# a16z/jolt

Measured on AMD Instinct MI355X. Metric: prover trace cycles/sec (sha3-shaped synthetic trace, sumcheck + HyperKZG hot path), higher is better.
Workload: dtype u256 (BN254 Fr / Fq, 8x u32 Montgomery limbs; integer, bit-exact)

## Files before the change

### jolt_amd/csrc/rw_matrix.hip

```cpp
#include <algorithm>
#include <vector>

#include "ctx.hpp"
#include "ints.hpp"
#include "onehot.hpp"
#include "poly_kernels.hip.h"

using namespace jolt;

int32_t jolt_internal_table_new(jolt_ctx* ctx, size_t len, jolt_table** out);
int32_t jolt_internal_bind(jolt_ctx* ctx, jolt_table* const* tables, size_t k, const Fr& r, int32_t order);
int32_t jolt_internal_eq_levels(jolt_ctx* ctx, const Fr* r, size_t n, const Fr& scale, std::vector<jolt_table*>* levels);
int32_t jolt_internal_ensure_scratch(jolt_ctx* ctx, size_t partials, size_t results);

namespace {

constexpr uint64_t kNoAccess = 0xFFFFFFFFFFFFFFFFull;

struct RwArrays {
    uint64_t* key;
    uint64_t *prev_u, *next_u;
    Fr *prev_f, *next_f;
    Fr *val, *ra;
    Fr* wa;
// ... 144 lines not shown
        sm[threadIdx.x] = v;
        __syncthreads();
        for (int off = 1; off < kBlock; off <<= 1) {
            uint64_t t = (int)threadIdx.x >= off ? sm[threadIdx.x - off] : 0ull;
            __syncthreads();
            sm[threadIdx.x] += t;
            __syncthreads();
        }
        if (i < nblocks) sums[i] = carry + sm[threadIdx.x] - v;
        __syncthreads();
        if (threadIdx.x == kBlock - 1) carry += sm[threadIdx.x];
        __syncthreads();
    }
    if (threadIdx.x == 0) total[0] = carry;
}
__global__ __launch_bounds__(kBlock) void k_scan_add(uint64_t* __restrict__ out, uint32_t n, const uint64_t* __restrict__ block_sums) {
    const uint32_t base = (blockIdx.x * kBlock + threadIdx.x) * kScanItems;
    const uint64_t add_ = block_sums[blockIdx.x];
#pragma unroll
    for (int k = 0; k < kScanItems; ++k)
        if (base + k < n) out[base + k] += add_;
}

__global__ __launch_bounds__(kBlock) void k_rw_cycle_match(const uint64_t* __restrict__ key, uint32_t n, uint32_t* __restrict__ sib_lb, uint32_t* __restrict__ matched,
                                                           uint64_t* __restrict__ flags) {
    uint32_t i = blockIdx.x * kBlock + threadIdx.x;
    if (i >= n) return;
    const uint64_t k = key[i], want = k ^ (1ull << 32);
    const uint32_t lb = lower_bound_near(key, n, want, i);
    const bool m = lb < n && key[lb] == want;
    const bool even = ((k >> 32) & 1) == 0;
    sib_lb[i] = lb;
    matched[i] = m ? 1u : 0u;
    flags[i] = ((even || !m) ? 1ull : 0ull) | ((even && m) ? (1ull << 32) : 0ull);
}

template <bool REG>
__global__ __launch_bounds__(kBlock) void k_rw_cycle_round(RwArrays a, uint32_t n, const uint32_t* __restrict__ sib_lb, const uint32_t* __restrict__ matched,
                                                           const Fr* __restrict__ inc, const Fr* __restrict__ e_out, const Fr* __restrict__ e_in, int in_bits, Fr gamma,
                                                           Fr* __restrict__ partials) {
    Fr acc[2] = {Fr::zero(), Fr::zero()};
    const uint32_t stride = gridDim.x * kBlock;
    for (uint32_t i = blockIdx.x * kBlock + threadIdx.x; i < n; i += stride) {
        const uint64_t k = a.key[i];
        const uint32_t row = (uint32_t)(k >> 32);
        const bool even = (row & 1) == 0, m = matched[i] != 0;
        if (!even && m) continue;
        const uint32_t pair = row >> 1;
        const Fr inc0 = ld_fr(inc + 2 * (size_t)pair), inc1 = sub(ld_fr(inc + 2 * (size_t)pair + 1), inc0);
        const Fr ra = ld_fr(a.ra + i), val = ld_fr(a.val + i);
        Fr q0, q1;
        if constexpr (REG) {
            const Fr wa = ld_fr(a.wa + i);
            if (even) {
                Fr ra_slope, wa_slope, val_slope;
                if (m) {
                    const uint32_t o = sib_lb[i];
// ... 17 lines not shown
            if (m) {
                const uint32_t o = sib_lb[i];
                ra_slope = sub(ld_fr(a.ra + o), ra);
                val_slope = sub(ld_fr(a.val + o), val);
            } else {
                ra_slope = neg(ra);
                val_slope = sub(fr_from_u64(a.next_u[i]), val);
            }
            q0 = mul(ra, slope_term(val, inc0, gamma));
            q1 = mul(ra_slope, slope_term(val_slope, inc1, gamma));
        } else {
            q0 = Fr::zero();
            q1 = mul(ra, slope_term(sub(val, fr_from_u64(a.prev_u[i])), inc1, gamma));
        }
        const Fr head = mul(ld_fr(e_out + (pair >> in_bits)), ld_fr(e_in + (pair & ((1u << in_bits) - 1))));
        acc[0] = add(acc[0], mul(head, q0));
        acc[1] = add(acc[1], mul(head, q1));
    }
    block_reduce_store<2>(acc, partials);
}

template <bool REG>
__global__ __launch_bounds__(kBlock) void k_rw_cycle_bind(RwArrays a, uint32_t n, const uint32_t* __restrict__ sib_lb, const uint32_t* __restrict__ matched,
                                                          const uint64_t* __restrict__ scan, Fr r, int shifted, RwArrays o) {
    uint32_t i = blockIdx.x * kBlock + threadIdx.x;
    if (i >= n) return;
    const uint64_t k = a.key[i];
    const uint32_t row = (uint32_t)(k >> 32), col = (uint32_t)k;
    const bool even = (row & 1) == 0, m = matched[i] != 0;
    if (!even && m) return;
    const uint64_t gkey = (uint64_t)(row & ~1u) << 32;
    const uint32_t gs = lower_bound_near(a.key, n, gkey, i), os = lower_bound_near(a.key, n, gkey | (1ull << 32), i);
    const uint64_t s_gs = gs < n ? scan[gs] : 0;
    const uint32_t out_base = (uint32_t)s_gs, m_gs = (uint32_t)(s_gs >> 32);
    const uint32_t lb = sib_lb[i];
    uint32_t pos;
    if (even) pos = out_base + (i - gs) + (lb - os) - ((uint32_t)(scan[i] >> 32) - m_gs);
    else pos = out_base + (i - os) + (lb - gs) - ((lb < n ? (uint32_t)(scan[lb] >> 32) : 0u) - m_gs);
    const Fr ra = ld_fr(a.ra + i), val = ld_fr(a.val + i);
    Fr nra, nval;
    uint64_t np, nn;
    auto lerp = [&](const Fr& lo, const Fr& hi) { return bind_pair(lo, hi, r, shifted); };
    if (even && m) {
        nra = lerp(ra, ld_fr(a.ra + lb));
        nval = lerp(val, ld_fr(a.val + lb));
        np = a.prev_u[i];
        nn = a.next_u[lb];
    } else if (even) {
        nra = lerp(ra, Fr::zero());
        nval = lerp(val, fr_from_u64(a.next_u[i]));
        np = a.prev_u[i];
        nn = a.next_u[i];
    } else {
        nra = lerp(Fr::zero(), ra);
        nval = lerp(fr_from_u64(a.prev_u[i]), val);
        np = a.prev_u[i];
        nn = a.next_u[i];
    }
    o.key[pos] = ((uint64_t)(row >> 1) << 32) | col;
    o.prev_u[pos] = np;
    o.next_u[pos] = nn;
    st_fr(o.ra + pos, nra);
    st_fr(o.val + pos, nval);
    if constexpr (REG) {
        const Fr wa = ld_fr(a.wa + i);
        st_fr(o.wa + pos, (even && m) ? lerp(wa, ld_fr(a.wa + lb)) : (even ? lerp(wa, Fr::zero()) : lerp(Fr::zero(), wa)));
    }
}

__global__ __launch_bounds__(kBlock) void k_rw_to_address_major(RwArrays a, uint32_t n) {
    uint32_t i = blockIdx.x * kBlock + threadIdx.x;
    if (i >= n) return;
    a.key[i] = (uint32_t)a.key[i];
    st_fr(a.prev_f + i, fr_from_u64(a.prev_u[i]));
    st_fr(a.next_f + i, fr_from_u64(a.next_u[i]));
}

__device__ __forceinline__ bool adr_partner(const uint64_t* __restrict__ key, uint32_t n, uint32_t i, uint32_t& other) {
    const uint64_t c = key[i];
    if ((c & 1) == 0) { other = i + 1; return i + 1 < n && key[i + 1] == c + 1; }
    other = i - 1;
    return i > 0 && key[i - 1] == c - 1;
}
__global__ __launch_bounds__(kBlock) void k_rw_address_flags(const uint64_t* __restrict__ key, uint32_t n, uint64_t* __restrict__ flags) {
    uint32_t i = blockIdx.x * kBlock + threadIdx.x;
    if (i >= n) return;
    uint32_t o;
    const bool m = adr_partner(key, n, i, o);
    flags[i] = ((key[i] & 1) == 0 || !m) ? 1ull : 0ull;
}
__global__ __launch_bounds__(kBlock) void k_rw_address_round(RwArrays a, uint32_t n, const Fr* __restrict__ val_init, const Fr* __restrict__ inc_scalar, Fr eq_eval,
                                                             Fr gamma, Fr* __restrict__ partials) {
    Fr acc[2] = {Fr::zero(), Fr::zero()};
    const Fr inc = ld_fr(inc_scalar);
    const uint32_t stride = gridDim.x * kBlock;
    for (uint32_t i = blockIdx.x * kBlock + threadIdx.x; i < n; i += stride) {
        uint32_t o;
        const bool m = adr_partner(a.key, n, i, o);
        const uint64_t c = a.key[i];
        const bool even = (c & 1) == 0;
        if (!even && m) continue;
        const Fr ra = ld_fr(a.ra + i), val = ld_fr(a.val + i);
        Fr s0, s2;
        if (even) {
            Fr ra2, val2;
            if (m) {
                const Fr ora = ld_fr(a.ra + o), oval = ld_fr(a.val + o);
                ra2 = sub(add(ora, ora), ra);
                val2 = sub(add(oval, oval), val);
            } else {
                const Fr cp = ld_fr(val_init + (c | 1));
                ra2 = neg(ra);
                val2 = sub(add(cp, cp), val);
            }
            s0 = mul(mul(eq_eval, ra), slope_term(val, inc, gamma));
            s2 = mul(mul(eq_eval, ra2), slope_term(val2, inc, gamma));
        } else {
            const Fr cp = ld_fr(val_init + (c & ~1ull));
            s0 = Fr::zero();
            s2 = mul(mul(eq_eval, add(ra, ra)), slope_term(sub(add(val, val), cp), inc, gamma));
        }
        acc[0] = add(acc[0], s0);
        acc[1] = add(acc[1], s2);
    }
    block_reduce_store<2>(acc, partials);
}
__global__ __launch_bounds__(kBlock) void k_rw_address_bind(RwArrays a, uint32_t n, const Fr* __restrict__ val_init, const uint64_t* __restrict__ scan, Fr r, int shifted,
                                                            RwArrays o) {
    uint32_t i = blockIdx.x * kBlock + threadIdx.x;
    if (i >= n) return;
    uint32_t p;
    const bool m = adr_partner(a.key, n, i, p);
    const uint64_t c = a.key[i];
    const bool even = (c & 1) == 0;
    if (!even && m) return;
    const uint32_t pos = (uint32_t)scan[i];
    auto lerp = [&](const Fr& lo, const Fr& hi) { return bind_pair(lo, hi, r, shifted); };
    const Fr ra = ld_fr(a.ra + i), val = ld_fr(a.val + i), pv = ld_fr(a.prev_f + i), nx = ld_fr(a.next_f + i);
    Fr nra, nval, npv, nnx;
    if (even && m) {
        nra = lerp(ra, ld_fr(a.ra + p));
        nval = lerp(val, ld_fr(a.val + p));
        npv = lerp(pv, ld_fr(a.prev_f + p));
        nnx = lerp(nx, ld_fr(a.next_f + p));
    } else if (even) {
        const Fr cp = ld_fr(val_init + (c | 1));
        nra = lerp(ra, Fr::zero());
        nval = lerp(val, cp);
        npv = lerp(pv, cp);
        nnx = lerp(nx, cp);
    } else {
        const Fr cp = ld_fr(val_init + (c & ~1ull));
        nra = lerp(Fr::zero(), ra);
        nval = lerp(cp, val);
        npv = lerp(cp, pv);
        nnx = lerp(cp, nx);
    }
    o.key[pos] = c >> 1;
    st_fr(o.ra + pos, nra);
    st_fr(o.val + pos, nval);
    st_fr(o.prev_f + pos, npv);
    st_fr(o.next_f + pos, nnx);
}

}

struct jolt_rw_matrix {
    jolt_ctx* ctx = nullptr;
    size_t log_t = 0, log_k = 0, round = 0;
    uint32_t n = 0, cap = 0;
    void* block = nullptr;
    RwArrays st[2];
    int cur = 0;
    uint32_t *sib_lb = nullptr, *matched = nullptr;
    uint64_t *flags = nullptr, *scan = nullptr, *block_sums = nullptr, *total = nullptr;
    uint64_t* h_total = nullptr;
    bool match_valid = false;
    bool registers = false;
    bool hold_row = false;
    std::vector<Fr> reg_ra, reg_wa, reg_val;
    Fr inc_scalar;
    jolt_table *inc = nullptr, *val_init = nullptr;
    Fr gamma;
    std::vector<Fr> w;
    Fr current_scalar;
    size_t out_len = 0, in_len = 0, e_out_bits = 0, e_in_bits = 0;
    std::vector<jolt_table*> e_out_cache, e_in_cache;
};

static int32_t rw_scan(jolt_rw_matrix* m, uint32_t n) {
    jolt_ctx* ctx = m->ctx;
    const uint32_t per = kBlock * kScanItems, nblocks = std::max<uint32_t>(1, (n + per - 1) / per);
    hipLaunchKernelGGL(k_scan_blocks, dim3(nblocks), dim3(kBlock), 0, ctx->stream, (const uint64_t*)m->flags, n, m->scan, m->block_sums);
    hipLaunchKernelGGL(k_scan_sums, dim3(1), dim3(kBlock), 0, ctx->stream, m->block_sums, nblocks, m->total);
    hipLaunchKernelGGL(k_scan_add, dim3(nblocks), dim3(kBlock), 0, ctx->stream, m->scan, n, (const uint64_t*)m->block_sums);
    JOLT_HIP_TRY(ctx, hipGetLastError());
    return JOLT_OK;
}
static int32_t rw_read_total(jolt_rw_matrix* m, uint32_t* out) {
    jolt_ctx* ctx = m->ctx;
    JOLT_HIP_TRY(ctx, hipMemcpyAsync(m->h_total, m->total, 8, hipMemcpyDeviceToHost, ctx->stream));
    JOLT_HIP_TRY(ctx, hipStreamSynchronize(ctx->stream));
    *out = (uint32_t)*m->h_total;
    return JOLT_OK;
}
static unsigned rw_grid(uint32_t n) { return std::max<unsigned>(1, (n + kBlock - 1) / kBlock); }
constexpr uint32_t kRwRoundMult = 4;

extern "C" int32_t jolt_rw_matrix_destroy(jolt_rw_matrix* m) {
    if (!m) return JOLT_OK;
    jolt_ctx* ctx = m->ctx;
    if (m->block) jolt_internal_dev_free(ctx, m->block);
    if (m->h_total) (void)hipHostFree(m->h_total);
    if (m->inc) jolt_table_free(ctx, m->inc);
    if (m->val_init) jolt_table_free(ctx, m->val_init);
    for (jolt_table* t : m->e_out_cache) jolt_table_free(ctx, t);
    for (jolt_table* t : m->e_in_cache) jolt_table_free(ctx, t);
    delete m;
    return JOLT_OK;
}

static int32_t rw_create_impl(jolt_ctx* ctx, const uint64_t* addresses, const uint64_t* pre_values, const uint64_t* post_values, bool resident, uint32_t resident_cap,
                              size_t cycles, const jolt_table* inc, const jolt_table* val_init, const jolt_fr_t* tau_low, const jolt_fr_t* gamma, jolt_rw_matrix** out) {
    if (!ctx || !addresses || !pre_values || !post_values || !inc || !val_init || !tau_low || !gamma || !out) return JOLT_ERR_INVALID_ARG;
    if (cycles < 2 || (cycles & (cycles - 1)) || cycles > ((size_t)1 << 31) || inc->len != cycles) return JOLT_ERR_SIZE_MISMATCH;
    const size_t K = val_init->len;
    if (K == 0 || (K & (K - 1)) || K > ((size_t)1 << 32)) return JOLT_ERR_SIZE_MISMATCH;
    for (size_t j = 0; j < cycles && !resident; ++j)
        if (addresses[j] != kNoAccess && addresses[j] >= K) { ctx->last_error = "RAM address outside the address space"; return JOLT_ERR_INVALID_ARG; }
    jolt_rw_matrix* m = new (std::nothrow) jolt_rw_matrix();
// ... 36 lines not shown
    if (s == JOLT_OK && hipHostMalloc((void**)&m->h_total, 64, hipHostMallocDefault) != hipSuccess) s = JOLT_ERR_HIP;
    if (s != JOLT_OK) { jolt_rw_matrix_destroy(m); return s; }
    char* base = (char*)m->block;
    for (int b = 0; b < 2; ++b) {
        m->st[b].key = (uint64_t*)(base + o_st[b][0]); m->st[b].prev_u = (uint64_t*)(base + o_st[b][1]); m->st[b].next_u = (uint64_t*)(base + o_st[b][2]);
        m->st[b].prev_f = (Fr*)(base + o_st[b][3]); m->st[b].next_f = (Fr*)(base + o_st[b][4]); m->st[b].val = (Fr*)(base + o_st[b][5]); m->st[b].ra = (Fr*)(base + o_st[b][6]);
        m->st[b].wa = (Fr*)(base + o_st[b][7]);
    }
    m->sib_lb = (uint32_t*)(base + o_sib); m->matched = (uint32_t*)(base + o_match); m->flags = (uint64_t*)(base + o_flags); m->scan = (uint64_t*)(base + o_scan);
    m->block_sums = (uint64_t*)(base + o_bs); m->total = (uint64_t*)(base + o_total);
    const uint64_t *d_addr = addresses, *d_pre = pre_values, *d_post = post_values;
    hipError_t e = hipSuccess;
    if (!resident) {
        uint64_t* up = (uint64_t*)(base + o_up);
        d_addr = up; d_pre = up + cycles; d_post = up + 2 * cycles;
        e = hipMemcpyAsync(up, addresses, cycles * 8, hipMemcpyHostToDevice, ctx->stream);
        if (e == hipSuccess) e = hipMemcpyAsync(up + cycles, pre_values, cycles * 8, hipMemcpyHostToDevice, ctx->stream);
        if (e == hipSuccess) e = hipMemcpyAsync(up + 2 * cycles, post_values, cycles * 8, hipMemcpyHostToDevice, ctx->stream);
    }
    if (e == hipSuccess) {
        hipLaunchKernelGGL(k_rw_access_flags, dim3(rw_grid(T)), dim3(kBlock), 0, ctx->stream, (const uint64_t*)d_addr, T, m->flags);
        e = hipGetLastError();
    }
    if (e == hipSuccess) s = rw_scan(m, T);
    if (e == hipSuccess && s == JOLT_OK) {
        hipLaunchKernelGGL(k_rw_build, dim3(rw_grid(T)), dim3(kBlock), 0, ctx->stream, (const uint64_t*)d_addr, (const uint64_t*)d_pre, (const uint64_t*)d_post, T,
                           (const uint64_t*)m->scan, m->st[0]);
        e = hipGetLastError();
    }
    if (e == hipSuccess && !resident) e = hipStreamSynchronize(ctx->stream);
    if (e != hipSuccess || s != JOLT_OK) {
        if (e != hipSuccess) { ctx->last_error = std::string("rw matrix: ") + hipGetErrorString(e); s = JOLT_ERR_HIP; }
        jolt_rw_matrix_destroy(m);
        return s;
    }
    m->n = cap;
    *out = m;
    return JOLT_OK;
}
extern "C" int32_t jolt_rw_matrix_create(jolt_ctx* ctx, const uint64_t* addresses, const uint64_t* pre_values, const uint64_t* post_values, size_t cycles,
                                         const jolt_table* inc, const jolt_table* val_init, const jolt_fr_t* tau_low, const jolt_fr_t* gamma, jolt_rw_matrix** out) {
    return rw_create_impl(ctx, addresses, pre_values, post_values, false, 0, cycles, inc, val_init, tau_low, gamma, out);
}
__global__ __launch_bounds__(kBlock) void k_rw_count_accesses(const uint64_t* __restrict__ addresses, uint32_t cycles, uint64_t K, uint32_t* __restrict__ counters) {
    __shared__ uint32_t s_hit[kBlock / 64], s_bad[kBlock / 64];
    uint32_t hit = 0, bad = 0;
    for (uint32_t j = blockIdx.x * kBlock + threadIdx.x; j < cycles; j += gridDim.x * kBlock) {
// ... 23 lines not shown
    if (cycles < 2 || cycles > ((size_t)1 << 31)) return JOLT_ERR_SIZE_MISMATCH;
    uint32_t* d_counters = nullptr;
    JOLT_TRY(jolt_internal_dev_alloc(ctx, 256, (void**)&d_counters));
    uint32_t h_counters[2] = {0, 0};
    hipError_t e = hipMemsetAsync(d_counters, 0, 8, ctx->stream);
    if (e == hipSuccess) {
        hipLaunchKernelGGL(k_rw_count_accesses, dim3(std::min<uint32_t>(rw_grid((uint32_t)cycles), (uint32_t)ctx->num_cus * 8)), dim3(kBlock), 0, ctx->stream, (const uint64_t*)addresses->data, (uint32_t)cycles,
                           (uint64_t)val_init->len, d_counters);
        e = hipGetLastError();
    }
    if (e == hipSuccess) e = hipMemcpyAsync(h_counters, d_counters, 8, hipMemcpyDeviceToHost, ctx->stream);
    if (e == hipSuccess) e = hipStreamSynchronize(ctx->stream);
    jolt_internal_dev_free(ctx, d_counters);
    if (e != hipSuccess) { ctx->last_error = std::string("rw matrix: ") + hipGetErrorString(e); return JOLT_ERR_HIP; }
    if (h_counters[1]) { ctx->last_error = "RAM address outside the address space"; return JOLT_ERR_INVALID_ARG; }
    return rw_create_impl(ctx, (const uint64_t*)addresses->data, (const uint64_t*)pre_values->data, (const uint64_t*)post_values->data, true, h_counters[0], cycles, inc,
                          val_init, tau_low, gamma, out);
}

static int32_t rw_ingest(jolt_rw_matrix* m, const Fr& r) {
    jolt_ctx* ctx = m->ctx;
    const int shifted = fr_low_limbs_zero(r) ? 1 : 0;
    RwArrays &a = m->st[m->cur], &o = m->st[1 - m->cur];
    if (m->round < m->log_t) {
        if (m->n) {
            if (!m->match_valid) {
                hipLaunchKernelGGL(k_rw_cycle_match, dim3(rw_grid(m->n)), dim3(kBlock), 0, ctx->stream, (const uint64_t*)a.key, m->n, m->sib_lb, m->matched, m->flags);
                JOLT_HIP_TRY(ctx, hipGetLastError());
            }
            JOLT_TRY(rw_scan(m, m->n));
            if (m->registers)
                hipLaunchKernelGGL(k_rw_cycle_bind<true>, dim3(rw_grid(m->n)), dim3(kBlock), 0, ctx->stream, a, m->n, (const uint32_t*)m->sib_lb, (const uint32_t*)m->matched,
                                   (const uint64_t*)m->scan, r, shifted, o);
            else
                hipLaunchKernelGGL(k_rw_cycle_bind<false>, dim3(rw_grid(m->n)), dim3(kBlock), 0, ctx->stream, a, m->n, (const uint32_t*)m->sib_lb, (const uint32_t*)m->matched,
                                   (const uint64_t*)m->scan, r, shifted, o);
            JOLT_HIP_TRY(ctx, hipGetLastError());
            JOLT_TRY(rw_read_total(m, &m->n));
            m->cur = 1 - m->cur;
        }
        m->match_valid = false;
        JOLT_TRY(jolt_internal_bind(ctx, &m->inc, 1, r, JOLT_ORDER_LOW_TO_HIGH));
        {
            const size_t nvar = m->log_t;
            size_t current_index = nvar - m->round;
            const Fr p = m->w[current_index - 1], prod = mul(p, r);
            m->current_scalar = mul(m->current_scalar, add(add(sub(sub(Fr::one(), p), r), prod), prod));
            current_index -= 1;
            if (nvar / 2 < current_index && m->e_in_bits > 0) m->e_in_bits -= 1;
            else if (0 < current_index && m->e_out_bits > 0) m->e_out_bits -= 1;
        }
        if (m->round == m->log_t - 1 && m->hold_row) {
        } else if (m->round == m->log_t - 1 && m->registers) {
            const size_t K = (size_t)1 << m->log_k;
            m->reg_ra.assign(K, Fr::zero());
            m->reg_wa.assign(K, Fr::zero());
            m->reg_val.assign(K, Fr::zero());
            const uint32_t n = m->n;
            if (n > K) { ctx->last_error = "registers matrix: more cells than registers after the cycle rounds"; return JOLT_ERR_INVALID_ARG; }
            std::vector<uint64_t> key(n);
            std::vector<Fr> ra(n), wa(n), val(n);
            const RwArrays& c = m->st[m->cur];
            hipError_t first = hipSuccess;
            auto copy = [&](void* dst, const void* src, size_t bytes) {
// ... 7 lines not shown
                copy(val.data(), c.val, (size_t)n * sizeof(Fr));
            }
            copy(&m->inc_scalar, m->inc->data(), sizeof(Fr));
            const hipError_t sync = hipStreamSynchronize(ctx->stream);
            JOLT_HIP_TRY(ctx, first);
            JOLT_HIP_TRY(ctx, sync);
            for (uint32_t i = 0; i < n; ++i) {
                const uint32_t col = (uint32_t)key[i];
                if ((key[i] >> 32) != 0 || col >= K) { ctx->last_error = "registers matrix: a cell outside the single bound row"; return JOLT_ERR_INVALID_ARG; }
                m->reg_ra[col] = ra[i]; m->reg_wa[col] = wa[i]; m->reg_val[col] = val[i];
            }
        } else if (m->round == m->log_t - 1 && m->n) {
            hipLaunchKernelGGL(k_rw_to_address_major, dim3(rw_grid(m->n)), dim3(kBlock), 0, ctx->stream, m->st[m->cur], m->n);
            JOLT_HIP_TRY(ctx, hipGetLastError());
        }
    } else if (m->registers) {
        for (std::vector<Fr>* t : {&m->reg_ra, &m->reg_wa, &m->reg_val}) {
            const size_t half = t->size() / 2;
            for (size_t y = 0; y < half; ++y) (*t)[y] = add((*t)[2 * y], mul(r, sub((*t)[2 * y + 1], (*t)[2 * y])));
            t->resize(half);
        }
    } else {
        if (m->n) {
            hipLaunchKernelGGL(k_rw_address_flags, dim3(rw_grid(m->n)), dim3(kBlock), 0, ctx->stream, (const uint64_t*)a.key, m->n, m->flags);
            JOLT_HIP_TRY(ctx, hipGetLastError());
            JOLT_TRY(rw_scan(m, m->n));
            hipLaunchKernelGGL(k_rw_address_bind, dim3(rw_grid(m->n)), dim3(kBlock), 0, ctx->stream, a, m->n, (const Fr*)m->val_init->data(), (const uint64_t*)m->scan, r,
                               shifted, o);
            JOLT_HIP_TRY(ctx, hipGetLastError());
            JOLT_TRY(rw_read_total(m, &m->n));
            m->cur = 1 - m->cur;
        }
        JOLT_TRY(jolt_internal_bind(ctx, &m->val_init, 1, r, JOLT_ORDER_LOW_TO_HIGH));
    }
    m->round += 1;
    return JOLT_OK;
}

extern "C" int32_t jolt_rw_matrix_prove_round(jolt_rw_matrix* m, const jolt_fr_t* bind, jolt_fr_t* evals_out, jolt_fr_t* aux_out) {
    if (!m || !evals_out) return JOLT_ERR_INVALID_ARG;
    jolt_ctx* ctx = m->ctx;
    if (m->registers) { ctx->last_error = "a registers handle: use jolt_registers_rw_prove_round (this entry point ignores the wa column)"; return JOLT_ERR_INVALID_ARG; }
    if (bind) {
        Fr r = fr_from_abi(bind);
        JOLT_REQUIRE(ctx, fr_is_canonical(r), "bind challenge is not a canonical Fr");
        if (m->round >= m->log_t + m->log_k) { ctx->last_error = "rw matrix already fully bound"; return JOLT_ERR_INVALID_ARG; }
        JOLT_TRY(rw_ingest(m, r));
    }
    if (m->round >= m->log_t + m->log_k) { ctx->last_error = "prove_round on a fully bound rw matrix"; return JOLT_ERR_INVALID_ARG; }
    const int grid = (int)std::max<uint32_t>(1, std::min<uint32_t>((m->n + kBlock - 1) / kBlock, (uint32_t)ctx->num_cus * kRwRoundMult));
    JOLT_TRY(jolt_internal_ensure_scratch(ctx, (size_t)grid * 2 + 8, 8));
    RwArrays& a = m->st[m->cur];
    Fr zero = Fr::zero();
    if (m->round < m->log_t) {
        if (m->n && !m->match_valid) {
            hipLaunchKernelGGL(k_rw_cycle_match, dim3(rw_grid(m->n)), dim3(kBlock), 0, ctx->stream, (const uint64_t*)a.key, m->n, m->sib_lb, m->matched, m->flags);
            JOLT_HIP_TRY(ctx, hipGetLastError());
            m->match_valid = true;
        }
        hipLaunchKernelGGL(k_rw_cycle_round<false>, dim3(grid), dim3(kBlock), 0, ctx->stream, a, m->n, (const uint32_t*)m->sib_lb, (const uint32_t*)m->matched,
                           (const Fr*)m->inc->data(), (const Fr*)m->e_out_cache[m->e_out_bits]->data(), (const Fr*)m->e_in_cache[m->e_in_bits]->data(), (int)m->e_in_bits,
                           m->gamma, ctx->d_partials);
        if (aux_out) {
            fr_to_abi(&aux_out[0], m->current_scalar);
            fr_to_abi(&aux_out[1], m->w[m->log_t - m->round - 1]);
            fr_to_abi(&aux_out[2], zero);
        }
    } else {
        hipLaunchKernelGGL(k_rw_address_round, dim3(grid), dim3(kBlock), 0, ctx->stream, a, m->n, (const Fr*)m->val_init->data(), (const Fr*)m->inc->data(),
                           m->current_scalar, m->gamma, ctx->d_partials);
        if (aux_out) for (int k = 0; k < 3; ++k) fr_to_abi(&aux_out[k], zero);
    }
    JOLT_HIP_TRY(ctx, hipGetLastError());
    hipLaunchKernelGGL(k_reduce_partials, dim3(1), dim3(kBlock), 0, ctx->stream, (const Fr*)ctx->d_partials, grid, 2, ctx->d_results);
    JOLT_HIP_TRY(ctx, hipGetLastError());
    JOLT_HIP_TRY(ctx, hipMemcpyAsync(ctx->h_results, ctx->d_results, 2 * sizeof(Fr), hipMemcpyDeviceToHost, ctx->stream));
    JOLT_HIP_TRY(ctx, hipStreamSynchronize(ctx->stream));
    std::memcpy(evals_out, ctx->h_results, 2 * sizeof(Fr));
    return JOLT_OK;
}

extern "C" int32_t jolt_rw_matrix_finish(jolt_rw_matrix* m, const jolt_fr_t* bind) {
    if (!m || !bind) return JOLT_ERR_INVALID_ARG;
    Fr r = fr_from_abi(bind);
    JOLT_REQUIRE(m->ctx, fr_is_canonical(r), "bind challenge is not a canonical Fr");
    if (m->round + 1 != m->log_t + m->log_k) { m->ctx->last_error = "finish_rounds before the last round"; return JOLT_ERR_INVALID_ARG; }
    return rw_ingest(m, r);
}

extern "C" int32_t jolt_rw_matrix_final_values(jolt_rw_matrix* m, jolt_fr_t* out) {
    if (!m || !out) return JOLT_ERR_INVALID_ARG;
    jolt_ctx* ctx = m->ctx;
    if (m->registers) { ctx->last_error = "a registers handle: use jolt_registers_rw_final_values (no val_init column here)"; return JOLT_ERR_INVALID_ARG; }
    if (m->round != m->log_t + m->log_k) return JOLT_ERR_NOT_FULLY_BOUND;
    Fr vals[3];
    if (m->n) {
        JOLT_HIP_TRY(ctx, hipMemcpyAsync(&vals[0], m->st[m->cur].ra, sizeof(Fr), hipMemcpyDeviceToHost, ctx->stream));
        JOLT_HIP_TRY(ctx, hipMemcpyAsync(&vals[1], m->st[m->cur].val, sizeof(Fr), hipMemcpyDeviceToHost, ctx->stream));
    } else {
        vals[0] = Fr::zero();
        JOLT_HIP_TRY(ctx, hipMemcpyAsync(&vals[1], m->val_init->data(), sizeof(Fr), hipMemcpyDeviceToHost, ctx->stream));
// ... 189 lines not shown
    while (((size_t)1 << m->log_k) < K) m->log_k++;
    m->gamma = fr_from_abi(gamma);
    m->w.resize(m->log_t);
    for (size_t i = 0; i < m->log_t; ++i) m->w[i] = fr_from_abi(&r_cycle[i]);
    m->current_scalar = Fr::one();
    int32_t s = fr_is_canonical(m->gamma) ? JOLT_OK : JOLT_ERR_INVALID_ARG;
    for (size_t i = 0; i < m->log_t && s == JOLT_OK; ++i) if (!fr_is_canonical(m->w[i])) s = JOLT_ERR_INVALID_ARG;
    const size_t split = m->log_t / 2, head_len = m->log_t - 1;
    m->out_len = std::min(split, head_len);
    m->in_len = head_len - m->out_len;
    m->e_out_bits = m->out_len;
    m->e_in_bits = m->in_len;
    if (s == JOLT_OK) s = jolt_internal_eq_levels(ctx, m->w.data(), m->out_len, Fr::one(), &m->e_out_cache);
    if (s == JOLT_OK) s = jolt_internal_eq_levels(ctx, m->w.data() + m->out_len, m->in_len, Fr::one(), &m->e_in_cache);
    if (s == JOLT_OK) s = jolt_table_clone(ctx, inc, &m->inc);
    const uint32_t T = (uint32_t)cycles;
    const size_t scan_len0 = T;
    uint64_t *d_flags0 = nullptr;
    if (s == JOLT_OK) s = jolt_internal_dev_alloc(ctx, (2 * scan_len0 + ((scan_len0 + kBlock * kScanItems - 1) / (kBlock * kScanItems) + 1) + 32) * 8, (void**)&d_flags0);
    if (s == JOLT_OK && hipHostMalloc((void**)&m->h_total, 64, hipHostMallocDefault) != hipSuccess) s = JOLT_ERR_HIP;
    if (s != JOLT_OK) { if (d_flags0) jolt_internal_dev_free(ctx, d_flags0); jolt_rw_matrix_destroy(m); return s; }
    m->flags = d_flags0; m->scan = d_flags0 + scan_len0; m->block_sums = m->scan + scan_len0; m->total = m->block_sums + ((scan_len0 + kBlock * kScanItems - 1) / (kBlock * kScanItems) + 1);
    hipLaunchKernelGGL(k_reg_count, dim3(rw_grid(T)), dim3(kBlock), 0, ctx->stream, (const uint8_t*)regs->idx, regs->wide, T, m->flags);
    s = hipGetLastError() == hipSuccess ? rw_scan(m, T) : JOLT_ERR_HIP;
    uint32_t cap = 0;
    if (s == JOLT_OK) s = rw_read_total(m, &cap);
    if (s != JOLT_OK) { jolt_internal_dev_free(ctx, d_flags0); m->flags = m->scan = m->block_sums = m->total = nullptr; jolt_rw_matrix_destroy(m); return s; }
    m->cap = std::max<uint32_t>(cap, 1);
    const size_t scan_len = std::max<size_t>(T, m->cap);
    size_t off = 0;
    auto take = [&](size_t bytes) { size_t o = off; off += (bytes + 255) & ~(size_t)255; return o; };
    size_t o_st[2][6];
    for (int b = 0; b < 2; ++b) {
        o_st[b][0] = take((size_t)m->cap * 8); o_st[b][1] = take((size_t)m->cap * 8); o_st[b][2] = take((size_t)m->cap * 8);
        o_st[b][3] = take((size_t)m->cap * 32); o_st[b][4] = take((size_t)m->cap * 32); o_st[b][5] = take((size_t)m->cap * 32);
    }
    const size_t o_sib = take((size_t)m->cap * 4), o_match = take((size_t)m->cap * 4), o_flags = take(scan_len * 8), o_scan = take(scan_len * 8),
                 o_bs = take(((scan_len + kBlock * kScanItems - 1) / (kBlock * kScanItems) + 1) * 8), o_total = take(256);
    s = jolt_internal_dev_alloc(ctx, off, &m->block);
    if (s != JOLT_OK) { jolt_internal_dev_free(ctx, d_flags0); m->flags = m->scan = m->block_sums = m->total = nullptr; jolt_rw_matrix_destroy(m); return s; }
    char* base = (char*)m->block;
    for (int b = 0; b < 2; ++b) {
        m->st[b].key = (uint64_t*)(base + o_st[b][0]); m->st[b].prev_u = (uint64_t*)(base + o_st[b][1]); m->st[b].next_u = (uint64_t*)(base + o_st[b][2]);
        m->st[b].val = (Fr*)(base + o_st[b][3]); m->st[b].ra = (Fr*)(base + o_st[b][4]); m->st[b].wa = (Fr*)(base + o_st[b][5]);
        m->st[b].prev_f = nullptr; m->st[b].next_f = nullptr;
    }
    const uint64_t* pos = m->scan;
    hipLaunchKernelGGL(k_reg_build, dim3(rw_grid(T)), dim3(kBlock), 0, ctx->stream, (const uint8_t*)regs->idx, regs->wide, (const uint64_t*)rs1_val->data, (const uint64_t*)rs2_val->data,
                       (const uint64_t*)rd_pre->data, (const uint64_t*)rd_post->data, T, pos, m->gamma, mul(m->gamma, m->gamma), m->st[0]);
// ... 1 lines not shown
    jolt_internal_dev_free(ctx, d_flags0);
    m->sib_lb = (uint32_t*)(base + o_sib); m->matched = (uint32_t*)(base + o_match); m->flags = (uint64_t*)(base + o_flags); m->scan = (uint64_t*)(base + o_scan);
    m->block_sums = (uint64_t*)(base + o_bs); m->total = (uint64_t*)(base + o_total);
    if (e != hipSuccess) { ctx->last_error = std::string("registers matrix: ") + hipGetErrorString(e); jolt_rw_matrix_destroy(m); return JOLT_ERR_HIP; }
    m->n = cap;
    *out = m;
    return JOLT_OK;
}

extern "C" int32_t jolt_registers_rw_prove_round(jolt_rw_matrix* m, const jolt_fr_t* bind, jolt_fr_t* evals_out, jolt_fr_t* aux_out) {
    if (!m || !evals_out || !m->registers) return JOLT_ERR_INVALID_ARG;
    jolt_ctx* ctx = m->ctx;
    if (bind) {
        Fr r = fr_from_abi(bind);
        JOLT_REQUIRE(ctx, fr_is_canonical(r), "bind challenge is not a canonical Fr");
        if (m->round >= m->log_t + m->log_k) { ctx->last_error = "registers matrix already fully bound"; return JOLT_ERR_INVALID_ARG; }
        JOLT_TRY(rw_ingest(m, r));
    }
    if (m->round >= m->log_t + m->log_k) { ctx->last_error = "prove_round on a fully bound registers matrix"; return JOLT_ERR_INVALID_ARG; }
    const Fr zero = Fr::zero();
    for (int k = 0; k < 4; ++k) fr_to_abi(&evals_out[k], zero);
    if (aux_out) for (int k = 0; k < 3; ++k) fr_to_abi(&aux_out[k], zero);
    if (m->round < m->log_t) {
        const int grid = (int)std::max<uint32_t>(1, std::min<uint32_t>((m->n + kBlock - 1) / kBlock, (uint32_t)ctx->num_cus * kRwRoundMult));
        JOLT_TRY(jolt_internal_ensure_scratch(ctx, (size_t)grid * 2 + 8, 8));
        RwArrays& a = m->st[m->cur];
        if (m->n && !m->match_valid) {
            hipLaunchKernelGGL(k_rw_cycle_match, dim3(rw_grid(m->n)), dim3(kBlock), 0, ctx->stream, (const uint64_t*)a.key, m->n, m->sib_lb, m->matched, m->flags);
            JOLT_HIP_TRY(ctx, hipGetLastError());
            m->match_valid = true;
        }
        hipLaunchKernelGGL(k_rw_cycle_round<true>, dim3(grid), dim3(kBlock), 0, ctx->stream, a, m->n, (const uint32_t*)m->sib_lb, (const uint32_t*)m->matched, (const Fr*)m->inc->data(),
                           (const Fr*)m->e_out_cache[m->e_out_bits]->data(), (const Fr*)m->e_in_cache[m->e_in_bits]->data(), (int)m->e_in_bits, m->gamma, ctx->d_partials);
        JOLT_HIP_TRY(ctx, hipGetLastError());
        hipLaunchKernelGGL(k_reduce_partials, dim3(1), dim3(kBlock), 0, ctx->stream, (const Fr*)ctx->d_partials, grid, 2, ctx->d_results);
        JOLT_HIP_TRY(ctx, hipGetLastError());
        JOLT_HIP_TRY(ctx, hipMemcpyAsync(ctx->h_results, ctx->d_results, 2 * sizeof(Fr), hipMemcpyDeviceToHost, ctx->stream));
        JOLT_HIP_TRY(ctx, hipStreamSynchronize(ctx->stream));
        std::memcpy(evals_out, ctx->h_results, 2 * sizeof(Fr));
        if (aux_out) {
            fr_to_abi(&aux_out[0], m->current_scalar);
            fr_to_abi(&aux_out[1], m->w[m->log_t - m->round - 1]);
        }
        return JOLT_OK;
    }
    Fr ev[4] = {zero, zero, zero, zero};
    const size_t half = m->reg_ra.size() / 2;
    for (size_t y = 0; y < half; ++y) {
        Fr ra_t = m->reg_ra[2 * y], wa_t = m->reg_wa[2 * y], val_t = m->reg_val[2 * y];
        const Fr ra_m = sub(m->reg_ra[2 * y + 1], ra_t), wa_m = sub(m->reg_wa[2 * y + 1], wa_t), val_m = sub(m->reg_val[2 * y + 1], val_t);
        for (int t = 0; t < 4; ++t) {
            ev[t] = add(ev[t], add(mul(wa_t, add(m->inc_scalar, val_t)), mul(ra_t, val_t)));
            ra_t = add(ra_t, ra_m); wa_t = add(wa_t, wa_m); val_t = add(val_t, val_m);
        }
    }
    for (int t = 0; t < 4; ++t) fr_to_abi(&evals_out[t], mul(m->current_scalar, ev[t]));
    return JOLT_OK;
}

extern "C" int32_t jolt_registers_rw_final_values(jolt_rw_matrix* m, jolt_fr_t* out) {
    if (!m || !out || !m->registers) return JOLT_ERR_INVALID_ARG;
    if (m->round != m->log_t + m->log_k) return JOLT_ERR_NOT_FULLY_BOUND;
// ... 27 lines not shown
```

Before: 12.07 million.

## Fuse RW compaction scan into round kernel and drop per-bind host sync

The match/flags kernel now also computes tile-local prefix counts with wave ballots. A single-block kernel both scans the tile totals and reduces the sumcheck partials, so one readback returns the evaluations together with the next compacted length. The bind step reuses this scan instead of running a separate multi-kernel scan plus a blocking total readback, which removes one host synchronization and several launches per round. In exchange the bind kernels do an extra indirection per scan lookup, and a single block now has to walk all tile totals serially.

```diff
diff --git a/jolt_amd/csrc/rw_matrix.hip b/jolt_amd/csrc/rw_matrix.hip
--- a/jolt_amd/csrc/rw_matrix.hip
+++ b/jolt_amd/csrc/rw_matrix.hip
@@ -190,17 +190,104 @@
         if (base + k < n) out[base + k] += add_;
 }
 
+__global__ __launch_bounds__(kBlock) void k_rw_scan_reduce(uint64_t* __restrict__ tiles, uint32_t ntiles, const Fr* __restrict__ partials, int nblocks, Fr* __restrict__ out) {
+    __shared__ uint64_t sm[kBlock];
+    __shared__ Fr sums[kBlock / 64];
+    const uint32_t per = (ntiles + kBlock - 1) / kBlock, lo = min(ntiles, threadIdx.x * per), hi = min(ntiles, lo + per);
+    uint64_t local = 0;
+    for (uint32_t i = lo; i < hi; ++i) local += tiles[i];
+    sm[threadIdx.x] = local;
+    __syncthreads();
+    for (int off = 1; off < kBlock; off <<= 1) {
+        uint64_t t = (int)threadIdx.x >= off ? sm[threadIdx.x - off] : 0ull;
+        __syncthreads();
+        sm[threadIdx.x] += t;
+        __syncthreads();
+    }
+    uint64_t run = sm[threadIdx.x] - local;
+    for (uint32_t i = lo; i < hi; ++i) {
+        const uint64_t v = tiles[i];
+        tiles[i] = run;
+        run += v;
+    }
+    if (threadIdx.x == 0) *reinterpret_cast<uint64_t*>(out + 2) = sm[kBlock - 1];
+    const int lane = threadIdx.x & 63, wave = threadIdx.x >> 6;
+    for (int t = 0; t < 2; ++t) {
+        Fr s = Fr::zero();
+        for (int b = threadIdx.x; b < nblocks; b += kBlock) s = add(s, ld_fr(partials + (size_t)b * 2 + t));
+#pragma unroll
+        for (int off = 32; off >= 1; off >>= 1) {
+            Fr o;
+#pragma unroll
+            for (int k = 0; k < 8; ++k) o.l[k] = __shfl_xor(s.l[k], off, 64);
+            s = add(s, o);
+        }
+        if (lane == 0) sums[wave] = s;
+        __syncthreads();
+        if (threadIdx.x == 0) {
+            Fr tot = sums[0];
+            for (int w = 1; w < kBlock / 64; ++w) tot = add(tot, sums[w]);
+            st_fr(out + t, tot);
+        }
+        __syncthreads();
+    }
+}
+
+constexpr uint32_t kRwTile = 1024;
+constexpr int kRwSub = kRwTile / kBlock;
+constexpr int kRwWaves = kBlock / 64;
+constexpr int kRwChunks = kRwSub * kRwWaves;
+
+__device__ __forceinline__ uint32_t rw_tile_scan(uint32_t out_bits, uint32_t me_bits, uint32_t* cnt, uint32_t (&pre)[kRwSub]) {
+    const uint32_t lane = threadIdx.x & 63, wave = threadIdx.x >> 6;
+    const uint64_t below = (1ull << lane) - 1;
+#pragma unroll
+    for (int s = 0; s < kRwSub; ++s) {
+        const uint64_t bo = __ballot((out_bits >> s) & 1), bm = __ballot((me_bits >> s) & 1);
+        pre[s] = (uint32_t)__popcll(bo & below) | ((uint32_t)__popcll(bm & below) << 16);
+        if (lane == 0) cnt[s * kRwWaves + wave] = (uint32_t)__popcll(bo) | ((uint32_t)__popcll(bm) << 16);
+    }
+    __syncthreads();
+    uint32_t total = 0;
+#pragma unroll
+    for (int c = 0; c < kRwChunks; ++c) {
+        const uint32_t v = cnt[c];
+#pragma unroll
+        for (int s = 0; s < kRwSub; ++s) pre[s] += (uint32_t)c < s * kRwWaves + wave ? v : 0u;
+        total += v;
+    }
+    return total;
+}
+__device__ __forceinline__ uint64_t rw_unpack_counts(uint32_t packed) { return (uint64_t)(packed & 0xFFFFu) | ((uint64_t)(packed >> 16) << 32); }
+__device__ __forceinline__ uint64_t rw_scan_at(const uint64_t* __restrict__ tile_prefix, const uint32_t* __restrict__ in_tile, uint32_t x) {
+    return tile_prefix[x / kRwTile] + rw_unpack_counts(in_tile[x]);
+}
+
 __global__ __launch_bounds__(kBlock) void k_rw_cycle_match(const uint64_t* __restrict__ key, uint32_t n, uint32_t* __restrict__ sib_lb, uint32_t* __restrict__ matched,
-                                                           uint64_t* __restrict__ flags) {
-    uint32_t i = blockIdx.x * kBlock + threadIdx.x;
-    if (i >= n) return;
-    const uint64_t k = key[i], want = k ^ (1ull << 32);
-    const uint32_t lb = lower_bound_near(key, n, want, i);
-    const bool m = lb < n && key[lb] == want;
-    const bool even = ((k >> 32) & 1) == 0;
-    sib_lb[i] = lb;
-    matched[i] = m ? 1u : 0u;
-    flags[i] = ((even || !m) ? 1ull : 0ull) | ((even && m) ? (1ull << 32) : 0ull);
+                                                           uint32_t* __restrict__ in_tile, uint64_t* __restrict__ tile_totals) {
+    __shared__ uint32_t s_cnt[kRwChunks];
+    const uint32_t first = blockIdx.x * kRwTile + threadIdx.x;
+    uint32_t out_bits = 0, me_bits = 0;
+#pragma unroll
+    for (int s = 0; s < kRwSub; ++s) {
+        const uint32_t i = first + s * kBlock;
+        if (i < n) {
+            const uint64_t k = key[i], want = k ^ (1ull << 32);
+            const uint32_t lb = lower_bound_near(key, n, want, i);
+            const bool m = lb < n && key[lb] == want;
+            const bool even = ((k >> 32) & 1) == 0;
+            sib_lb[i] = lb;
+            matched[i] = m ? 1u : 0u;
+            out_bits |= ((even || !m) ? 1u : 0u) << s;
+            me_bits |= ((even && m) ? 1u : 0u) << s;
+        }
+    }
+    uint32_t pre[kRwSub];
+    const uint32_t total = rw_tile_scan(out_bits, me_bits, s_cnt, pre);
+#pragma unroll
+    for (int s = 0; s < kRwSub; ++s)
+        if (first + s * kBlock < n) in_tile[first + s * kBlock] = pre[s];
+    if (threadIdx.x == 0) tile_totals[blockIdx.x] = rw_unpack_counts(total);
 }
 
 template <bool REG>
@@ -264,7 +351,7 @@
 
 template <bool REG>
 __global__ __launch_bounds__(kBlock) void k_rw_cycle_bind(RwArrays a, uint32_t n, const uint32_t* __restrict__ sib_lb, const uint32_t* __restrict__ matched,
-                                                          const uint64_t* __restrict__ scan, Fr r, int shifted, RwArrays o) {
+                                                          const uint64_t* __restrict__ tile_prefix, const uint32_t* __restrict__ in_tile, Fr r, int shifted, RwArrays o) {
     uint32_t i = blockIdx.x * kBlock + threadIdx.x;
     if (i >= n) return;
     const uint64_t k = a.key[i];
@@ -273,12 +360,12 @@
     if (!even && m) return;
     const uint64_t gkey = (uint64_t)(row & ~1u) << 32;
     const uint32_t gs = lower_bound_near(a.key, n, gkey, i), os = lower_bound_near(a.key, n, gkey | (1ull << 32), i);
-    const uint64_t s_gs = gs < n ? scan[gs] : 0;
+    const uint64_t s_gs = gs < n ? rw_scan_at(tile_prefix, in_tile, gs) : 0;
     const uint32_t out_base = (uint32_t)s_gs, m_gs = (uint32_t)(s_gs >> 32);
     const uint32_t lb = sib_lb[i];
     uint32_t pos;
-    if (even) pos = out_base + (i - gs) + (lb - os) - ((uint32_t)(scan[i] >> 32) - m_gs);
-    else pos = out_base + (i - os) + (lb - gs) - ((lb < n ? (uint32_t)(scan[lb] >> 32) : 0u) - m_gs);
+    if (even) pos = out_base + (i - gs) + (lb - os) - ((uint32_t)(rw_scan_at(tile_prefix, in_tile, i) >> 32) - m_gs);
+    else pos = out_base + (i - os) + (lb - gs) - ((lb < n ? (uint32_t)(rw_scan_at(tile_prefix, in_tile, lb) >> 32) : 0u) - m_gs);
     const Fr ra = ld_fr(a.ra + i), val = ld_fr(a.val + i);
     Fr nra, nval;
     uint64_t np, nn;
@@ -324,12 +411,25 @@
     other = i - 1;
     return i > 0 && key[i - 1] == c - 1;
 }
-__global__ __launch_bounds__(kBlock) void k_rw_address_flags(const uint64_t* __restrict__ key, uint32_t n, uint64_t* __restrict__ flags) {
-    uint32_t i = blockIdx.x * kBlock + threadIdx.x;
-    if (i >= n) return;
-    uint32_t o;
-    const bool m = adr_partner(key, n, i, o);
-    flags[i] = ((key[i] & 1) == 0 || !m) ? 1ull : 0ull;
+__global__ __launch_bounds__(kBlock) void k_rw_address_counts(const uint64_t* __restrict__ key, uint32_t n, uint32_t* __restrict__ in_tile, uint64_t* __restrict__ tile_totals) {
+    __shared__ uint32_t s_cnt[kRwChunks];
+    const uint32_t first = blockIdx.x * kRwTile + threadIdx.x;
+    uint32_t out_bits = 0;
+#pragma unroll
+    for (int s = 0; s < kRwSub; ++s) {
+        const uint32_t i = first + s * kBlock;
+        if (i < n) {
+            uint32_t o;
+            const bool m = adr_partner(key, n, i, o);
+            out_bits |= (((key[i] & 1) == 0 || !m) ? 1u : 0u) << s;
+        }
+    }
+    uint32_t pre[kRwSub];
+    const uint32_t total = rw_tile_scan(out_bits, 0u, s_cnt, pre);
+#pragma unroll
+    for (int s = 0; s < kRwSub; ++s)
+        if (first + s * kBlock < n) in_tile[first + s * kBlock] = pre[s];
+    if (threadIdx.x == 0) tile_totals[blockIdx.x] = rw_unpack_counts(total);
 }
 __global__ __launch_bounds__(kBlock) void k_rw_address_round(RwArrays a, uint32_t n, const Fr* __restrict__ val_init, const Fr* __restrict__ inc_scalar, Fr eq_eval,
                                                              Fr gamma, Fr* __restrict__ partials) {
@@ -367,8 +467,8 @@
     }
     block_reduce_store<2>(acc, partials);
 }
-__global__ __launch_bounds__(kBlock) void k_rw_address_bind(RwArrays a, uint32_t n, const Fr* __restrict__ val_init, const uint64_t* __restrict__ scan, Fr r, int shifted,
-                                                            RwArrays o) {
+__global__ __launch_bounds__(kBlock) void k_rw_address_bind(RwArrays a, uint32_t n, const Fr* __restrict__ val_init, const uint64_t* __restrict__ tile_prefix,
+                                                            const uint32_t* __restrict__ in_tile, Fr r, int shifted, RwArrays o) {
     uint32_t i = blockIdx.x * kBlock + threadIdx.x;
     if (i >= n) return;
     uint32_t p;
@@ -376,7 +476,7 @@
     const uint64_t c = a.key[i];
     const bool even = (c & 1) == 0;
     if (!even && m) return;
-    const uint32_t pos = (uint32_t)scan[i];
+    const uint32_t pos = (uint32_t)rw_scan_at(tile_prefix, in_tile, i);
     auto lerp = [&](const Fr& lo, const Fr& hi) { return bind_pair(lo, hi, r, shifted); };
     const Fr ra = ld_fr(a.ra + i), val = ld_fr(a.val + i), pv = ld_fr(a.prev_f + i), nx = ld_fr(a.next_f + i);
     Fr nra, nval, npv, nnx;
@@ -411,13 +511,14 @@
     jolt_ctx* ctx = nullptr;
     size_t log_t = 0, log_k = 0, round = 0;
     uint32_t n = 0, cap = 0;
+    uint32_t n_next = 0;
+    bool round_valid = false;
     void* block = nullptr;
     RwArrays st[2];
     int cur = 0;
     uint32_t *sib_lb = nullptr, *matched = nullptr;
     uint64_t *flags = nullptr, *scan = nullptr, *block_sums = nullptr, *total = nullptr;
     uint64_t* h_total = nullptr;
-    bool match_valid = false;
     bool registers = false;
     bool hold_row = false;
     std::vector<Fr> reg_ra, reg_wa, reg_val;
@@ -430,7 +531,7 @@
     std::vector<jolt_table*> e_out_cache, e_in_cache;
 };
 
-static int32_t rw_scan(jolt_rw_matrix* m, uint32_t n) {
+static int32_t rw_build_scan(jolt_rw_matrix* m, uint32_t n) {
     jolt_ctx* ctx = m->ctx;
     const uint32_t per = kBlock * kScanItems, nblocks = std::max<uint32_t>(1, (n + per - 1) / per);
     hipLaunchKernelGGL(k_scan_blocks, dim3(nblocks), dim3(kBlock), 0, ctx->stream, (const uint64_t*)m->flags, n, m->scan, m->block_sums);
@@ -439,7 +540,7 @@
     JOLT_HIP_TRY(ctx, hipGetLastError());
     return JOLT_OK;
 }
-static int32_t rw_read_total(jolt_rw_matrix* m, uint32_t* out) {
+static int32_t rw_build_count(jolt_rw_matrix* m, uint32_t* out) {
     jolt_ctx* ctx = m->ctx;
     JOLT_HIP_TRY(ctx, hipMemcpyAsync(m->h_total, m->total, 8, hipMemcpyDeviceToHost, ctx->stream));
     JOLT_HIP_TRY(ctx, hipStreamSynchronize(ctx->stream));
@@ -448,6 +549,48 @@
 }
 static unsigned rw_grid(uint32_t n) { return std::max<unsigned>(1, (n + kBlock - 1) / kBlock); }
 constexpr uint32_t kRwRoundMult = 4;
+static uint32_t* rw_in_tile(jolt_rw_matrix* m) { return reinterpret_cast<uint32_t*>(m->flags); }
+static uint64_t* rw_tiles(jolt_rw_matrix* m) { return m->scan; }
+
+static int32_t rw_round(jolt_rw_matrix* m, Fr* ev) {
+    jolt_ctx* ctx = m->ctx;
+    m->round_valid = true;
+    if (!m->n) {
+        ev[0] = ev[1] = Fr::zero();
+        m->n_next = 0;
+        return JOLT_OK;
+    }
+    const uint32_t ntiles = (m->n + kRwTile - 1) / kRwTile;
+    const uint32_t grid = std::max<uint32_t>(1, std::min<uint32_t>((m->n + kBlock - 1) / kBlock, (uint32_t)ctx->num_cus * kRwRoundMult));
+    JOLT_TRY(jolt_internal_ensure_scratch(ctx, (size_t)grid * 2 + 8, 8));
+    RwArrays& a = m->st[m->cur];
+    if (m->round >= m->log_t) {
+        hipLaunchKernelGGL(k_rw_address_counts, dim3(ntiles), dim3(kBlock), 0, ctx->stream, (const uint64_t*)a.key, m->n, rw_in_tile(m), rw_tiles(m));
+        hipLaunchKernelGGL(k_rw_address_round, dim3(grid), dim3(kBlock), 0, ctx->stream, a, m->n, (const Fr*)m->val_init->data(), (const Fr*)m->inc->data(), m->current_scalar,
+                           m->gamma, ctx->d_partials);
+    } else {
+        hipLaunchKernelGGL(k_rw_cycle_match, dim3(ntiles), dim3(kBlock), 0, ctx->stream, (const uint64_t*)a.key, m->n, m->sib_lb, m->matched, rw_in_tile(m), rw_tiles(m));
+        if (m->registers)
+            hipLaunchKernelGGL(k_rw_cycle_round<true>, dim3(grid), dim3(kBlock), 0, ctx->stream, a, m->n, (const uint32_t*)m->sib_lb, (const uint32_t*)m->matched,
+                               (const Fr*)m->inc->data(), (const Fr*)m->e_out_cache[m->e_out_bits]->data(), (const Fr*)m->e_in_cache[m->e_in_bits]->data(), (int)m->e_in_bits,
+                               m->gamma, ctx->d_partials);
+        else
+            hipLaunchKernelGGL(k_rw_cycle_round<false>, dim3(grid), dim3(kBlock), 0, ctx->stream, a, m->n, (const uint32_t*)m->sib_lb, (const uint32_t*)m->matched,
+                               (const Fr*)m->inc->data(), (const Fr*)m->e_out_cache[m->e_out_bits]->data(), (const Fr*)m->e_in_cache[m->e_in_bits]->data(), (int)m->e_in_bits,
+                               m->gamma, ctx->d_partials);
+    }
+    JOLT_HIP_TRY(ctx, hipGetLastError());
+    hipLaunchKernelGGL(k_rw_scan_reduce, dim3(1), dim3(kBlock), 0, ctx->stream, rw_tiles(m), ntiles, (const Fr*)ctx->d_partials, (int)grid, ctx->d_results);
+    JOLT_HIP_TRY(ctx, hipGetLastError());
+    JOLT_HIP_TRY(ctx, hipMemcpyAsync(ctx->h_results, ctx->d_results, 2 * sizeof(Fr) + 8, hipMemcpyDeviceToHost, ctx->stream));
+    JOLT_HIP_TRY(ctx, hipStreamSynchronize(ctx->stream));
+    ev[0] = ctx->h_results[0];
+    ev[1] = ctx->h_results[1];
+    uint64_t total;
+    std::memcpy(&total, ctx->h_results + 2, 8);
+    m->n_next = (uint32_t)total;
+    return JOLT_OK;
+}
 
 extern "C" int32_t jolt_rw_matrix_destroy(jolt_rw_matrix* m) {
     if (!m) return JOLT_OK;
@@ -530,7 +673,7 @@
         hipLaunchKernelGGL(k_rw_access_flags, dim3(rw_grid(T)), dim3(kBlock), 0, ctx->stream, (const uint64_t*)d_addr, T, m->flags);
         e = hipGetLastError();
     }
-    if (e == hipSuccess) s = rw_scan(m, T);
+    if (e == hipSuccess) s = rw_build_scan(m, T);
     if (e == hipSuccess && s == JOLT_OK) {
         hipLaunchKernelGGL(k_rw_build, dim3(rw_grid(T)), dim3(kBlock), 0, ctx->stream, (const uint64_t*)d_addr, (const uint64_t*)d_pre, (const uint64_t*)d_post, T,
                            (const uint64_t*)m->scan, m->st[0]);
@@ -600,24 +743,21 @@
     jolt_ctx* ctx = m->ctx;
     const int shifted = fr_low_limbs_zero(r) ? 1 : 0;
     RwArrays &a = m->st[m->cur], &o = m->st[1 - m->cur];
+    Fr unused[2];
     if (m->round < m->log_t) {
         if (m->n) {
-            if (!m->match_valid) {
-                hipLaunchKernelGGL(k_rw_cycle_match, dim3(rw_grid(m->n)), dim3(kBlock), 0, ctx->stream, (const uint64_t*)a.key, m->n, m->sib_lb, m->matched, m->flags);
-                JOLT_HIP_TRY(ctx, hipGetLastError());
-            }
-            JOLT_TRY(rw_scan(m, m->n));
+            if (!m->round_valid) JOLT_TRY(rw_round(m, unused));
             if (m->registers)
                 hipLaunchKernelGGL(k_rw_cycle_bind<true>, dim3(rw_grid(m->n)), dim3(kBlock), 0, ctx->stream, a, m->n, (const uint32_t*)m->sib_lb, (const uint32_t*)m->matched,
-                                   (const uint64_t*)m->scan, r, shifted, o);
+                                   (const uint64_t*)rw_tiles(m), (const uint32_t*)rw_in_tile(m), r, shifted, o);
             else
                 hipLaunchKernelGGL(k_rw_cycle_bind<false>, dim3(rw_grid(m->n)), dim3(kBlock), 0, ctx->stream, a, m->n, (const uint32_t*)m->sib_lb, (const uint32_t*)m->matched,
-                                   (const uint64_t*)m->scan, r, shifted, o);
+                                   (const uint64_t*)rw_tiles(m), (const uint32_t*)rw_in_tile(m), r, shifted, o);
             JOLT_HIP_TRY(ctx, hipGetLastError());
-            JOLT_TRY(rw_read_total(m, &m->n));
+            m->n = m->n_next;
             m->cur = 1 - m->cur;
         }
-        m->match_valid = false;
+        m->round_valid = false;
         JOLT_TRY(jolt_internal_bind(ctx, &m->inc, 1, r, JOLT_ORDER_LOW_TO_HIGH));
         {
             const size_t nvar = m->log_t;
@@ -671,15 +811,14 @@
         }
     } else {
         if (m->n) {
-            hipLaunchKernelGGL(k_rw_address_flags, dim3(rw_grid(m->n)), dim3(kBlock), 0, ctx->stream, (const uint64_t*)a.key, m->n, m->flags);
+            if (!m->round_valid) JOLT_TRY(rw_round(m, unused));
+            hipLaunchKernelGGL(k_rw_address_bind, dim3(rw_grid(m->n)), dim3(kBlock), 0, ctx->stream, a, m->n, (const Fr*)m->val_init->data(), (const uint64_t*)rw_tiles(m),
+                               (const uint32_t*)rw_in_tile(m), r, shifted, o);
             JOLT_HIP_TRY(ctx, hipGetLastError());
-            JOLT_TRY(rw_scan(m, m->n));
-            hipLaunchKernelGGL(k_rw_address_bind, dim3(rw_grid(m->n)), dim3(kBlock), 0, ctx->stream, a, m->n, (const Fr*)m->val_init->data(), (const uint64_t*)m->scan, r,
-                               shifted, o);
-            JOLT_HIP_TRY(ctx, hipGetLastError());
-            JOLT_TRY(rw_read_total(m, &m->n));
+            m->n = m->n_next;
             m->cur = 1 - m->cur;
         }
+        m->round_valid = false;
         JOLT_TRY(jolt_internal_bind(ctx, &m->val_init, 1, r, JOLT_ORDER_LOW_TO_HIGH));
     }
     m->round += 1;
@@ -697,35 +836,17 @@
         JOLT_TRY(rw_ingest(m, r));
     }
     if (m->round >= m->log_t + m->log_k) { ctx->last_error = "prove_round on a fully bound rw matrix"; return JOLT_ERR_INVALID_ARG; }
-    const int grid = (int)std::max<uint32_t>(1, std::min<uint32_t>((m->n + kBlock - 1) / kBlock, (uint32_t)ctx->num_cus * kRwRoundMult));
-    JOLT_TRY(jolt_internal_ensure_scratch(ctx, (size_t)grid * 2 + 8, 8));
-    RwArrays& a = m->st[m->cur];
-    Fr zero = Fr::zero();
-    if (m->round < m->log_t) {
-        if (m->n && !m->match_valid) {
-            hipLaunchKernelGGL(k_rw_cycle_match, dim3(rw_grid(m->n)), dim3(kBlock), 0, ctx->stream, (const uint64_t*)a.key, m->n, m->sib_lb, m->matched, m->flags);
-            JOLT_HIP_TRY(ctx, hipGetLastError());
-            m->match_valid = true;
-        }
-        hipLaunchKernelGGL(k_rw_cycle_round<false>, dim3(grid), dim3(kBlock), 0, ctx->stream, a, m->n, (const uint32_t*)m->sib_lb, (const uint32_t*)m->matched,
-                           (const Fr*)m->inc->data(), (const Fr*)m->e_out_cache[m->e_out_bits]->data(), (const Fr*)m->e_in_cache[m->e_in_bits]->data(), (int)m->e_in_bits,
-                           m->gamma, ctx->d_partials);
-        if (aux_out) {
+    Fr ev[2];
+    JOLT_TRY(rw_round(m, ev));
+    std::memcpy(evals_out, ev, 2 * sizeof(Fr));
+    if (aux_out) {
+        const Fr zero = Fr::zero();
+        for (int k = 0; k < 3; ++k) fr_to_abi(&aux_out[k], zero);
+        if (m->round < m->log_t) {
             fr_to_abi(&aux_out[0], m->current_scalar);
             fr_to_abi(&aux_out[1], m->w[m->log_t - m->round - 1]);
-            fr_to_abi(&aux_out[2], zero);
-        }
-    } else {
-        hipLaunchKernelGGL(k_rw_address_round, dim3(grid), dim3(kBlock), 0, ctx->stream, a, m->n, (const Fr*)m->val_init->data(), (const Fr*)m->inc->data(),
-                           m->current_scalar, m->gamma, ctx->d_partials);
-        if (aux_out) for (int k = 0; k < 3; ++k) fr_to_abi(&aux_out[k], zero);
-    }
-    JOLT_HIP_TRY(ctx, hipGetLastError());
-    hipLaunchKernelGGL(k_reduce_partials, dim3(1), dim3(kBlock), 0, ctx->stream, (const Fr*)ctx->d_partials, grid, 2, ctx->d_results);
-    JOLT_HIP_TRY(ctx, hipGetLastError());
-    JOLT_HIP_TRY(ctx, hipMemcpyAsync(ctx->h_results, ctx->d_results, 2 * sizeof(Fr), hipMemcpyDeviceToHost, ctx->stream));
-    JOLT_HIP_TRY(ctx, hipStreamSynchronize(ctx->stream));
-    std::memcpy(evals_out, ctx->h_results, 2 * sizeof(Fr));
+        }
+    }
     return JOLT_OK;
 }
 
@@ -961,9 +1082,9 @@
     if (s != JOLT_OK) { if (d_flags0) jolt_internal_dev_free(ctx, d_flags0); jolt_rw_matrix_destroy(m); return s; }
     m->flags = d_flags0; m->scan = d_flags0 + scan_len0; m->block_sums = m->scan + scan_len0; m->total = m->block_sums + ((scan_len0 + kBlock * kScanItems - 1) / (kBlock * kScanItems) + 1);
     hipLaunchKernelGGL(k_reg_count, dim3(rw_grid(T)), dim3(kBlock), 0, ctx->stream, (const uint8_t*)regs->idx, regs->wide, T, m->flags);
-    s = hipGetLastError() == hipSuccess ? rw_scan(m, T) : JOLT_ERR_HIP;
+    s = hipGetLastError() == hipSuccess ? rw_build_scan(m, T) : JOLT_ERR_HIP;
     uint32_t cap = 0;
-    if (s == JOLT_OK) s = rw_read_total(m, &cap);
+    if (s == JOLT_OK) s = rw_build_count(m, &cap);
     if (s != JOLT_OK) { jolt_internal_dev_free(ctx, d_flags0); m->flags = m->scan = m->block_sums = m->total = nullptr; jolt_rw_matrix_destroy(m); return s; }
     m->cap = std::max<uint32_t>(cap, 1);
     const size_t scan_len = std::max<size_t>(T, m->cap);
@@ -1011,22 +1132,9 @@
     for (int k = 0; k < 4; ++k) fr_to_abi(&evals_out[k], zero);
     if (aux_out) for (int k = 0; k < 3; ++k) fr_to_abi(&aux_out[k], zero);
     if (m->round < m->log_t) {
-        const int grid = (int)std::max<uint32_t>(1, std::min<uint32_t>((m->n + kBlock - 1) / kBlock, (uint32_t)ctx->num_cus * kRwRoundMult));
-        JOLT_TRY(jolt_internal_ensure_scratch(ctx, (size_t)grid * 2 + 8, 8));
-        RwArrays& a = m->st[m->cur];
-        if (m->n && !m->match_valid) {
-            hipLaunchKernelGGL(k_rw_cycle_match, dim3(rw_grid(m->n)), dim3(kBlock), 0, ctx->stream, (const uint64_t*)a.key, m->n, m->sib_lb, m->matched, m->flags);
-            JOLT_HIP_TRY(ctx, hipGetLastError());
-            m->match_valid = true;
-        }
-        hipLaunchKernelGGL(k_rw_cycle_round<true>, dim3(grid), dim3(kBlock), 0, ctx->stream, a, m->n, (const uint32_t*)m->sib_lb, (const uint32_t*)m->matched, (const Fr*)m->inc->data(),
-                           (const Fr*)m->e_out_cache[m->e_out_bits]->data(), (const Fr*)m->e_in_cache[m->e_in_bits]->data(), (int)m->e_in_bits, m->gamma, ctx->d_partials);
-        JOLT_HIP_TRY(ctx, hipGetLastError());
-        hipLaunchKernelGGL(k_reduce_partials, dim3(1), dim3(kBlock), 0, ctx->stream, (const Fr*)ctx->d_partials, grid, 2, ctx->d_results);
-        JOLT_HIP_TRY(ctx, hipGetLastError());
-        JOLT_HIP_TRY(ctx, hipMemcpyAsync(ctx->h_results, ctx->d_results, 2 * sizeof(Fr), hipMemcpyDeviceToHost, ctx->stream));
-        JOLT_HIP_TRY(ctx, hipStreamSynchronize(ctx->stream));
-        std::memcpy(evals_out, ctx->h_results, 2 * sizeof(Fr));
+        Fr ev[2];
+        JOLT_TRY(rw_round(m, ev));
+        std::memcpy(evals_out, ev, 2 * sizeof(Fr));
         if (aux_out) {
             fr_to_abi(&aux_out[0], m->current_scalar);
             fr_to_abi(&aux_out[1], m->w[m->log_t - m->round - 1]);
```

Result: no change. 12.05 million (-0.1%).
